# sandyz1000/face-landmark-detector

Hardware: AMD Instinct MI355X
Metric: faces/sec (whole node), 256x256 batch inference: fused preprocess + FCN-8 forward + softmax + top-4 landmark decode + similarity/alignment warp (higher is better)
Workload: dtype f32; 1 GPU; BASELINE configs[1]: batch=64/GPU 256x256x3 uint8 crops, fcn_8(68) vanilla encoder fp32, random-init weights (seed 2), decode top-4 thresh 0, align to 256x256; global_batch=64, parallelism=dp1

## Files before the change

face-landmark-detector_amd/build.py:

```python
from __future__ import annotations

import concurrent.futures
import hashlib
import os
import shutil
import subprocess
import sys

HERE = os.path.dirname(os.path.abspath(__file__))
ROOT = os.path.dirname(HERE)
CSRC = os.path.join(HERE, "csrc")
INCLUDE = os.path.join(ROOT, "include")
OBJ_DIR = os.path.join(HERE, "csrc", "build")
LIB_PATH = os.path.join(HERE, "libflm_hip.so")

SOURCES = [
    "flm_api.hip",
    "flm_pack.hip",
    "flm_enc1.hip",
    "flm_igemm.hip",
    "flm_igemm_bf16.hip",
    "flm_conv3_halo.hip",
    "flm_score1x1.hip",
    "flm_tail_bf16.hip",
    "flm_convt.hip",
    "flm_up3_wreg.hip",
    "flm_decode.hip",
    "flm_cand.hip",
    "flm_misc.hip",
    "flm_frames.hip",
    "flm_mobile.hip",
]
FLAGS = ["--offload-arch=gfx950", "-O3", "-fPIC", "-std=c++17", "-ffp-contract=off",
         "-Wall", "-Wno-unused-function", "-I", INCLUDE, "-I", CSRC]


FILE_FLAGS = {"flm_enc1.hip": ["-mllvm", "-amdgpu-mfma-vgpr-form"]}


def _hipcc() -> str:
    for c in (shutil.which("hipcc"), "/opt/rocm/bin/hipcc"):
        if c and os.path.exists(c):
            return c
    raise RuntimeError("hipcc not found: the HIP extension cannot be built")


def _stamp(paths) -> str:
    h = hashlib.sha256()
    h.update(" ".join(FLAGS).encode())
    h.update(repr(sorted(FILE_FLAGS.items())).encode())
    for p in sorted(paths):
        with open(p, "rb") as f:
            h.update(p.encode())
            h.update(f.read())
    return h.hexdigest()


def build(force: bool = False, verbose: bool = True, extra_flags=()) -> str:
    os.makedirs(OBJ_DIR, exist_ok=True)
    headers = [os.path.join(CSRC, f) for f in os.listdir(CSRC) if f.endswith(".h")] + \
              [os.path.join(INCLUDE, f) for f in os.listdir(INCLUDE) if f.endswith(".h")]
    srcs = [os.path.join(CSRC, s) for s in SOURCES]
    stamp = _stamp(srcs + headers) + " ".join(extra_flags)
    stamp_file = os.path.join(OBJ_DIR, "stamp.txt")
    if not force and os.path.exists(LIB_PATH) and os.path.exists(stamp_file) and open(stamp_file).read() == stamp:
        return LIB_PATH
    hipcc = _hipcc()

    def compile_one(src):
        obj = os.path.join(OBJ_DIR, os.path.basename(src) + ".o")
        cmd = [hipcc, *FLAGS, *FILE_FLAGS.get(os.path.basename(src), []), *extra_flags, "-c", src, "-o", obj]
        r = subprocess.run(cmd, capture_output=True, text=True)
        if r.returncode != 0:
            raise RuntimeError("hipcc failed on %s:\n%s\n%s" % (src, r.stdout, r.stderr))
        if verbose and r.stderr.strip():
            sys.stderr.write(r.stderr)
        return obj
# ... 17 lines not shown
```

face-landmark-detector_amd/csrc/flm_api.hip:

```cpp
#include <cstdarg>
#include <cstdio>
#include <cstring>

#include "flm_common.h"

namespace flm {

static thread_local char g_err[512] = "";

void set_error(const char* fmt, ...) {
  va_list ap;
  va_start(ap, fmt);
  vsnprintf(g_err, sizeof(g_err), fmt, ap);
  va_end(ap);
}

int hip_fail(hipError_t e, const char* what) {
  set_error("HIP error %d (%s) at %s", (int)e, hipGetErrorString(e), what);
  return FLM_ERR_HIP;
}

struct ProfRec {
  const char* name;
  hipEvent_t a, b;
// ... 92 lines not shown
    if (fc_bytes > W.splitk_bytes) W.splitk_bytes = fc_bytes;
  }
  if (n <= 4) {
    const size_t enc3_bytes = sizeof(float) * 4 * (size_t)4 * (h / 4) * (w / 4) * 256;
    if (enc3_bytes > W.splitk_bytes) W.splitk_bytes = enc3_bytes;
  }
  W.splitk = take(cur, W.splitk_bytes);
  W.oh = h + (A.fcn32 ? 32 : 8);
  W.ow = w + (A.fcn32 ? 32 : 8);
  W.probs = SIZE_MAX;
  W.decode = SIZE_MAX;
  W.sub = W.tau = W.cand = W.cand_cnt = SIZE_MAX;
  W.cand_cap = 0;
  if (out_mode == FLM_OUT_LANDMARKS) {
    W.probs = take(cur, sizeof(float) * (size_t)n * W.oh * W.ow * C);
    W.decode = take(cur, decode_ws_bytes(n, W.oh, W.ow, C, decode_mode, n_points));
    if (landmark_candidates_enabled(co, g, A.fcn32, decode_mode, n_points, W.oh, W.ow)) {
      const int h3 = h / 8, w3 = w / 8;
      W.sub = take(cur, sizeof(unsigned) * (size_t)n * convt_sample_slots(g, h3, w3, cand_sub_for(co, n_points, g.bf16 != 0)) * 16 * g.MT);
      W.tau = take(cur, sizeof(float) * (size_t)n * C);
      W.cand_cap = (int)align_up((size_t)C * 64 * n_points * 4 / co.cap_div, 64);
      if (W.cand_cap < 64) W.cand_cap = 64;
      W.cand = take(cur, sizeof(unsigned long long) * (size_t)n * W.cand_cap);
      W.cand_cnt = take(cur, sizeof(unsigned) * ((size_t)n + 1));
    }
  }
  W.total = cur;
  return W;
}

static int check_fcn8_shape(int n, int h, int w, int C, int dtype) {
  if (dtype != FLM_F32 && dtype != FLM_BF16) {
    set_error("fcn8: unknown dtype %d (FLM_F32 = 0, FLM_BF16 = 1)", dtype);
    return FLM_ERR_UNSUPPORTED;
  }
  if (n <= 0 || h <= 0 || w <= 0 || (h % 32) || (w % 32)) {
    set_error("fcn8: input must be [N>0, H, W, 3] with H and W multiples of 32 (got n=%d h=%d w=%d)", n, h, w);
    return FLM_ERR_SHAPE;
  }
  if (C < 1 || C > kMaxClasses) {
    set_error("fcn8: n_classes must be in [1,%d] (got %d)", kMaxClasses, C);
    return FLM_ERR_SHAPE;
  }
  if (n > (1 << 24) || h > (1 << 15) || w > (1 << 15) || (long long)n * (h + 32) * (w + 32) * C >= (1ll << 40)) {
    set_error("fcn8: batch too large (n=%d h=%d w=%d: at most 2^40 output values per call)", n, h, w);
    return FLM_ERR_SHAPE;
  }
  return FLM_OK;
}

static int conv_layer(hipStream_t s, const char* blob, const ConvPack& c, const void* x, void* y, int n, int h,
                      int w, int relu, int pool, int posmajor, int dtype, int out_f32 = 0,
                      float* splitk_ws = nullptr, size_t splitk_bytes = 0, int stride = 1,
                      const void* res = nullptr) {
  IgemmDesc d;
  d.bf16 = dtype == FLM_BF16;
  d.out_f32 = out_f32;
  d.stride = stride;
  d.res = res;
  d.splitk_ws = splitk_ws;
  d.splitk_ws_bytes = splitk_bytes;
  d.x = x;
  d.wt = blob + c.w;
  d.scale = reinterpret_cast<const float*>(blob + c.scale);
  d.shift = reinterpret_cast<const float*>(blob + c.shift);
  d.y = y;
  d.n = n; d.h = h; d.w = w; d.cin = c.cin;
  d.cout = c.cout; d.coutpad = c.coutpad; d.ldc = c.cout;
  d.kh = c.kh; d.kw = c.kw; d.pad = c.pad;
  d.relu = relu; d.pool = pool; d.posmajor = posmajor;
  return launch_igemm(s, d);
}

}

using namespace flm;

extern "C" {

int flm_abi_version(void) { return FLM_ABI_VERSION; }

int flm_debug_query(const char* key, int arg) {
  if (key && !strcmp(key, "igemm_occupancy")) return igemm_occupancy((size_t)arg);
  return -1;
}

int flm_set_tuning(const char* key, int value) {
  if (!key) return FLM_ERR_ARG;
  if (!strcmp(key, "none")) return FLM_OK;
  if (!strcmp(key, "bf16_big_tiles")) {
    flm::igemm_bf16_big_enable(value);
    return FLM_OK;
  }
  if (!strcmp(key, "f32_two_level")) {
    flm::igemm_f32_group(value ? 0 : -1);
    return FLM_OK;
  }
  if (!strcmp(key, "f32_lean_tile")) {
    flm::igemm_f32_lean_enable(value);
    return FLM_OK;
  }
  if (!strcmp(key, "bf16_mfma16")) {
    flm::igemm_bf16_big_m16(value);
    return FLM_OK;
  }
  if (!strcmp(key, "bf16_halo_mfma16")) {
    flm::conv3_halo_m16(value);
    return FLM_OK;
  }
  if (!strcmp(key, "bf16_lds_dma")) {
    flm::igemm_bf16_big_dma(value);
    return FLM_OK;
  }
  if (!strcmp(key, "landmark_candidates") || !strcmp(key, "candidate_sub_phases") || !strcmp(key, "candidate_cap_div")) {
    set_error("flm_set_tuning: '%s' changes the workspace layout and is a per-call option now: pass flm_forward_opts to "
              "flm_fcn_workspace_bytes_opts / flm_fcn_forward_opts", key);
    return FLM_ERR_ARG;
  }
  if (!strcmp(key, "up3_cand8")) {
    if (value < 0 || value > 7) {
      set_error("flm_set_tuning: up3_cand8 must be in [0,7]");
      return FLM_ERR_ARG;
    }
    flm::convt_cand8_enable(value);
    return FLM_OK;
  }
  if (!strcmp(key, "up3_cand8_rows")) {
    if (value < 0 || value > 8 || (value & (value - 1))) {
      set_error("flm_set_tuning: up3_cand8_rows must be 0, 1, 2, 4 or 8");
      return FLM_ERR_ARG;
    }
    flm::convt_cand8_rows(value);
    return FLM_OK;
  }
  if (!strcmp(key, "up3_wreg")) {
    if (value < 0 || value > 1) {
      set_error("flm_set_tuning: up3_wreg must be 0 or 1");
      return FLM_ERR_ARG;
    }
    flm::convt_wreg_enable(value);
    return FLM_OK;
  }
  if (!strcmp(key, "bf16_score1x1")) {
    flm::score1x1_enable(value);
    return FLM_OK;
  }
  if (!strcmp(key, "bf16_fused_tail")) {
    flm::tail_fused_enable(value);
    return FLM_OK;
  }
  if (!strcmp(key, "decode_lds_dma")) {
    flm::decode_dma_enable(value);
    return FLM_OK;
  }
  if (!strcmp(key, "posmajor_order")) {
    flm::igemm_posperm_enable(value);
    return FLM_OK;
  }
  if (!strcmp(key, "warp_rows")) {
    if (value != 0 && value != 1 && value != 4) {
      set_error("flm_set_tuning: warp_rows must be 0, 1 or 4");
      return FLM_ERR_ARG;
    }
    flm::warp_rows_enable(value);
    return FLM_OK;
  }
  if (!strcmp(key, "bf16_conv3_halo")) {
    flm::conv3_halo_enable(value);
    return FLM_OK;
  }
  if (!strcmp(key, "bf16_group_n")) {
    if (value < 0 || value > 32 || (value & (value - 1))) {
      set_error("flm_set_tuning: bf16_group_n must be 0 or a power of two <= 32");
      return FLM_ERR_ARG;
    }
    flm::igemm_bf16_group_n(value);
    return FLM_OK;
  }
  set_error("flm_set_tuning: unknown key '%s'", key);
  return FLM_ERR_ARG;
}

int flm_profile_enable(int max_records) {
  if (g_prof) return FLM_OK;
  if (max_records <= 0 || max_records > (1 << 20)) {
    set_error("flm_profile_enable: bad record count");
    return FLM_ERR_ARG;
  }
  g_prof = new ProfRec[max_records];
  for (int i = 0; i < max_records; ++i) {
    FLM_HIP(hipEventCreate(&g_prof[i].a));
    FLM_HIP(hipEventCreate(&g_prof[i].b));
  }
  g_prof_cap = max_records;
  g_prof_n = 0;
  return FLM_OK;
}

int flm_profile_reset(void) {
  g_prof_n = 0;
  return FLM_OK;
// ... 216 lines not shown
      case ENC_MB_CONV1:
        rc = launch_mb_conv1(s, xin, in_format, n, hi, wi, w0, sc0, sh0, yout, bf);
        break;
      case ENC_RN_CONV1:
        rc = launch_rn_conv1(s, xin, in_format, n, hi, wi, w0, sc0, sh0, yout, bf);
        break;
      case ENC_MAXPOOL3:
        rc = launch_maxpool3(s, xin, n, hi, wi, e.cin, yout, bf);
        break;
      case ENC_MB_DW:
        rc = launch_mb_depthwise(s, xin, n, hi, wi, e.cin, e.stride, w0, sc0, sh0, yout, bf);
        break;
      case ENC_CONV3:
        rc = conv_layer(s, blob, L.enc[i], xin, yout, n, hi, wi,  1, e.pool, 0, dtype, 0,
                        reinterpret_cast<float*>(ws + W.splitk), W.splitk_bytes);
        break;
      case ENC_MB_PW:
        if (L.enc[i].cin != e.cin) {
          int pn = n, ph = hi, pw = wi;
          if (!(pw & 1)) pw >>= 1;
          else if (!(ph & 1)) ph >>= 1;
          else if (!(pn & 1)) pn >>= 1;
          else {
            set_error("flm_fcn_forward: the paired pointwise conv needs an even number of pixels per batch");
            rc = FLM_ERR_SHAPE;
            break;
          }
          rc = conv_layer(s, blob, L.enc[i], xin, yout, pn, ph, pw,  2, 0, 0, dtype);
        } else {
          rc = conv_layer(s, blob, L.enc[i], xin, yout, n, hi, wi,  2, 0, 0, dtype);
        }
        break;
      case ENC_CONV:
        rc = conv_layer(s, blob, L.enc[i], xin, yout, n, hi, wi, e.relu, 0, 0, dtype, 0, nullptr, 0, e.stride,
                        e.res >= 0 ? ws + W.act[e.res] : nullptr);
        break;
      default:
        set_error("flm_fcn_forward: unknown encoder layer kind %d", e.kind);
        rc = FLM_ERR_ARG;
    }
    if (rc) return rc;
  }
  const int h5 = h / 32, w5 = w / 32, h4 = h / 16, w4 = w / 16, h3 = h / 8, w3 = w / 8;
  { ProfScope ps(s, "fc6");
  rc = conv_layer(s, blob, L.fc6, f[4], fc6, n, h5, w5, 1, 0,  1, dtype, 0,
                  reinterpret_cast<float*>(ws + W.splitk), W.splitk_bytes); }
  if (rc) return rc;
  { ProfScope ps(s, "fc7");
  rc = conv_layer(s, blob, L.fc7, fc6, fc7, n, h5, w5, 1, 0, 0, dtype, 0,
                  reinterpret_cast<float*>(ws + W.splitk), W.splitk_bytes); }
  if (rc) return rc;
  { ProfScope ps(s, "score5");
  rc = conv_layer(s, blob, L.score5, fc7, score5, n, h5, w5, 0, 0, 0, dtype,  1,
                  reinterpret_cast<float*>(ws + W.splitk), W.splitk_bytes); }
  if (rc) return rc;
  ConvTDesc t;
  t.g = L.g;
  t.n = n;
  if (!fcn32) {
  { ProfScope ps(s, "score4");
  rc = conv_layer(s, blob, L.score4, f[3], fuse4, n, h4, w4, 0, 0, 0, dtype, 1); }
  if (rc) return rc;
  const bool fuse_seg = bf && L.g.C == 68 && L.score3.cin == 256 && L.score3.kh == 1;
  int fused_seg = 0;
  if (!fuse_seg) {
  { ProfScope ps(s, "score3");
  rc = conv_layer(s, blob, L.score3, f[2], seg, n, h3, w3, 0, 0, 0, dtype, 1); }
  if (rc) return rc;
  }
  t.x = score5; t.wf = blob + L.up5; t.skip = fuse4; t.y = fuse4;
  t.hi = h5; t.wi = w5; t.ho = h4; t.wo = w4; t.s = 2; t.ldy = L.g.Cp; t.epilogue = 0;
  { ProfScope ps(s, "up5");
  rc = launch_convt(s, t); }
  if (rc) return rc;
  if (fuse_seg) {
    ProfScope ps(s, "seg_fused");
    fused_seg = launch_seg_fused_bf16(s, fuse4, blob + L.up4, f[2], blob + L.score3.w,
                                      reinterpret_cast<const float*>(blob + L.score3.scale),
                                      reinterpret_cast<const float*>(blob + L.score3.shift), seg, n, h4, w4, L.g.C, L.g.Cp,
                                      L.g.G, L.score3.cin, L.score3.coutpad);
    if (fused_seg < 0) return fused_seg;
  }
  if (fuse_seg && !fused_seg) {
    ProfScope ps(s, "score3");
    rc = conv_layer(s, blob, L.score3, f[2], seg, n, h3, w3, 0, 0, 0, dtype, 1);
    if (rc) return rc;
  }
  t.x = fuse4; t.wf = blob + L.up4; t.skip = seg; t.y = seg;
  t.hi = h4; t.wi = w4; t.ho = h3; t.wo = w3;
  if (!fused_seg) {
  { ProfScope ps(s, "up4");
  rc = launch_convt(s, t); }
  if (rc) return rc;
  }
  }
  t.wf = blob + L.up3; t.skip = nullptr; t.ho = W.oh; t.wo = W.ow; t.ldy = C;
  if (fcn32) { t.x = score5; t.hi = h5; t.wi = w5; t.s = 32; }
  else { t.x = seg; t.hi = h3; t.wi = w3; t.s = 8; }
  if (out_mode == FLM_OUT_LOGITS || out_mode == FLM_OUT_PROBS) {
    t.y = out_dev;
    t.epilogue = (out_mode == FLM_OUT_PROBS) ? 1 : 0;
    if (out_mode == FLM_OUT_LOGITS && (C & 3)) {
      set_error("flm_fcn8_forward: FLM_OUT_LOGITS needs n_classes %% 4 == 0");
      return FLM_ERR_UNSUPPORTED;
    }
    ProfScope ps(s, "up3");
    return launch_convt(s, t);
  }
  if (out_mode == FLM_OUT_CLASSMAP) {
    t.y = out_dev;
    t.epilogue = 2;
    ProfScope ps(s, "up3");
    return launch_convt(s, t);
  }
  float* probs = reinterpret_cast<float*>(ws + W.probs);
  const unsigned* gate = nullptr;
  if (W.cand != SIZE_MAX) {
    float* sub = reinterpret_cast<float*>(ws + W.sub);
    float* tau = reinterpret_cast<float*>(ws + W.tau);
    unsigned* cnt = reinterpret_cast<unsigned*>(ws + W.cand_cnt);
    unsigned long long* cand = reinterpret_cast<unsigned long long*>(ws + W.cand);
    FLM_HIP(hipMemsetAsync(cnt, 0, sizeof(unsigned) * ((size_t)n + 1), s));
    ConvTDesc ts = t;
    ts.y = sub; ts.epilogue = 4; ts.sub = cand_sub_for(co, n_points, L.g.bf16 != 0);
    { ProfScope ps(s, "up3_sub");
    rc = launch_convt(s, ts); }
    if (rc) return rc;
    { ProfScope ps(s, "tau");
    rc = launch_cand_tau(s, reinterpret_cast<const unsigned*>(sub), n, convt_sample_slots(L.g, t.hi, t.wi, cand_sub_for(co, n_points, L.g.bf16 != 0)), 16 * L.g.MT, C,
                         n_points, tau); }
    if (rc) return rc;
    ConvTDesc tc = t;
    tc.y = nullptr; tc.epilogue = 3; tc.tau = tau; tc.cand = cand; tc.cand_cnt = cnt; tc.cand_cap = W.cand_cap;
    tc.scratch = probs; tc.scratch_bytes = sizeof(float) * (size_t)n * W.oh * W.ow * C;
    { ProfScope ps(s, "up3");
    rc = launch_convt(s, tc); }
    if (rc) return rc;
    { ProfScope ps(s, "decode");
    rc = launch_cand_merge(s, cand, cnt, n, W.ow, C, n_points, thresh, W.cand_cap, static_cast<double*>(out_dev)); }
    if (rc) return rc;
    gate = cnt + n;
    t.gate = gate;
  }
// ... 173 lines not shown
```

face-landmark-detector_amd/csrc/flm_common.h:

```cpp
#pragma once

#include <hip/hip_runtime.h>
#include <stddef.h>
#include <stdint.h>

#include <atomic>
#include <mutex>

#include "flm.h"

namespace flm {

void set_error(const char* fmt, ...);
int hip_fail(hipError_t e, const char* what);

#define FLM_HIP(call)                                            \
  do {                                                           \
    hipError_t e_ = (call);                                      \
    if (e_ != hipSuccess) return ::flm::hip_fail(e_, #call);     \
  } while (0)

#define FLM_LAUNCH_CHECK(what)                                   \
  do {                                                           \
    hipError_t e_ = hipGetLastError();                           \
// ... 74 lines not shown
struct Fcn8Pack {
  size_t enc1_w;
  size_t enc1_scale, enc1_shift;
  ConvPack enc[kMaxEnc];
  ConvPack fc6, fc7, score5, score4, score3;
  size_t up5, up4, up3;
  ConvTGeom g;
  int dtype;
  int arch;
  ArchSpec spec;
  size_t total;
};
Fcn8Pack fcn8_pack_layout(int C, int dtype, int arch = 0);

struct Fcn8Ws {
  size_t act[kMaxEnc];
  size_t f[5];
  size_t fc6, fc7, score5, fuse4, seg;
  size_t splitk;
  size_t splitk_bytes;
  size_t probs;
  size_t decode;
  size_t sub, tau, cand, cand_cnt;
  int cand_cap;
  size_t total;
  int oh, ow;
};
Fcn8Ws fcn8_ws_layout(int n, int h, int w, int C, int dtype, int out_mode, int decode_mode, int n_points,
                      int arch = 0, const flm_forward_opts* opts = nullptr);

int launch_pack_fcn(hipStream_t s, const flm_fcn_params& p, int C, const Fcn8Pack& L, char* blob);

int launch_enc1(hipStream_t s, const void* x, int in_format, int n, int h, int w, const float* w1p,
                const float* scale, const float* shift, void* f1, int out_bf16, int pool);

struct IgemmDesc {
  const void* x;
  const void* wt;
  const float* scale;
  const float* shift;
  void* y;
  int bf16;
  int out_f32;
  int n, h, w, cin;
  int cout;
  int coutpad;
  int ldc;
  int kh, kw, pad;
  int relu, pool, posmajor;
  int stride;
  const void* res;
  float* splitk_ws;
  size_t splitk_ws_bytes;
};
int launch_igemm(hipStream_t s, const IgemmDesc& d);
int igemm_occupancy(size_t lds_bytes);
void igemm_f32_group(int steps);
void igemm_f32_lean_enable(int on);
void igemm_bf16_big_enable(int on);
void igemm_bf16_group_n(int gn);
void igemm_bf16_big_dma(int on);
void igemm_bf16_big_m16(int on);
void conv3_halo_enable(int on);
void conv3_halo_m16(int on);
void score1x1_enable(int on);
void tail_fused_enable(int on);
void decode_dma_enable(int on);
void warp_rows_enable(int on);
void igemm_posperm_enable(int on);
int launch_seg_fused_bf16(hipStream_t s, const float* fuse4, const void* w4_packed, const void* f3, const void* w3,
                          const float* scale3, const float* shift3, float* seg, int n, int h4, int w4d, int C, int Cp,
                          int G, int cin3, int coutpad3);

struct ConvTDesc {
  const float* x;
  const void* wf;
  const float* skip;
  void* y;
  int n, hi, wi;
  int ho, wo;
  int s;
  int ldy;
  int epilogue;
  ConvTGeom g;
  int sub = 0;
  const float* tau = nullptr;
  unsigned long long* cand = nullptr;
  unsigned* cand_cnt = nullptr;
  int cand_cap = 0;
  const unsigned* gate = nullptr;
  void* scratch = nullptr;
  size_t scratch_bytes = 0;
};
int launch_convt(hipStream_t s, const ConvTDesc& d);
int convt_candidates_supported(const ConvTGeom& g);
__host__ __device__ inline int convt_share_layout(const ConvTGeom& g, int s) {
  return g.C == 68 && (g.bf16 ? g.G == 9 : g.G == 17) && (s % 4) == 0;
}
int convt_sample_slots(const ConvTGeom& g, int hi, int wi, int sub);
void convt_cand8_enable(int mask);
void convt_cand8_rows(int rpw);
void convt_wreg_enable(int on);
int launch_cand_tau(hipStream_t s, const unsigned* wave_max, int n, int slots, int ld, int l, int n_points, float* tau);

int launch_mb_conv1(hipStream_t s, const void* x, int in_format, int n, int h, int w, const float* wgt,
                    const float* scale, const float* shift, void* y, int bf16);
int launch_mb_depthwise(hipStream_t s, const void* x, int n, int h, int w, int c, int stride, const float* wgt,
                        const float* scale, const float* shift, void* y, int bf16);
int launch_rn_conv1(hipStream_t s, const void* x, int in_format, int n, int h, int w, const float* wgt,
                    const float* scale, const float* shift, void* y, int bf16);
int launch_maxpool3(hipStream_t s, const void* x, int n, int h, int w, int c, void* y, int bf16);

size_t decode_ws_bytes(int n, int h, int w, int l, int mode, int n_points);
int launch_decode(hipStream_t s, const float* hm, int n, int h, int w, int l, int mode, int n_points, float thresh,
                  double* out, void* ws, size_t ws_bytes, const unsigned* gate = nullptr);
size_t decode_sweep_ws_bytes(int n, int h, int w, int l, const int* modes, int n_modes);
int launch_decode_sweep(hipStream_t s, const float* hm, int n, int h, int w, int l, const int* modes, int n_modes,
                        float thresh, double* out, void* ws, size_t ws_bytes);
int launch_gaussian_heatmaps(hipStream_t s, const double* kp, int n, int l, int h, int w, double two_sigma_sq,
                             float* out);
int launch_cand_merge(hipStream_t s, const unsigned long long* cand, unsigned* cand_cnt, int n, int w, int l,
                      int n_points, float thresh, int cap, double* out);

int launch_preprocess(hipStream_t s, const uint8_t* img, int n, int h, int w, int norm, float* out);
int launch_similarity(hipStream_t s, const double* lm, const double* tmpl, int n, int k, double sx, double sy, float* m);
// ... 20 lines not shown
```

face-landmark-detector_amd/csrc/flm_igemm.hip:

```cpp
#include <type_traits>
#include <vector>

#include "flm_igemm_args.h"

#ifndef FLM_IGEMM_VAR
#define FLM_IGEMM_VAR 0
#endif

namespace flm {

typedef float f32x16 __attribute__((ext_vector_type(16)));
typedef __bf16 bf16x8 __attribute__((ext_vector_type(8)));

constexpr int BM = 128, BN = 128, BK = 32;
constexpr int TILE_F = BM * BK;

__device__ __forceinline__ int swz(int row, int chunk) { return row * BK + ((chunk ^ ((row >> 1) & 7)) << 2); }

__device__ __forceinline__ float f4c(const float4& v, int i) { return i == 0 ? v.x : (i == 1 ? v.y : (i == 2 ? v.z : v.w)); }

template <bool BF, int IDX>
__device__ __forceinline__ void mfma_slot(const float4& a0, const float4& a1, const float4& b0, const float4& b1,
                                          f32x16& c00, f32x16& c01, f32x16& c10, f32x16& c11) {
  if constexpr (BF) {
// ... 674 lines not shown
    for (int s = 0; s < ksplit; ++s) v += part[(size_t)s * total + i];
    v = fmaf(v, scale[c], shift[c]);
    if (relu) v = fmaxf(v, 0.f);
    if (out_bf16) reinterpret_cast<unsigned short*>(y)[i] = f2bf(v);
    else reinterpret_cast<float*>(y)[i] = v;
  }
}

__global__ void splitk_reduce_pool_kernel(const float* __restrict__ part, const float* __restrict__ scale,
                                          const float* __restrict__ shift, void* __restrict__ y, int M, int ldc, int cout,
                                          int ksplit, int relu, float relu_max, int out_bf16) {
  const size_t total = (size_t)(M >> 2) * ldc, plane = (size_t)M * ldc;
  for (size_t i = (size_t)blockIdx.x * blockDim.x + threadIdx.x; i < total; i += (size_t)gridDim.x * blockDim.x) {
    const int c = (int)(i % ldc);
    if (c >= cout) continue;
    const size_t q = i / ldc;
    float best = -3.402823466e38f;
#pragma unroll
    for (int e = 0; e < 4; ++e) {
      float v = 0.f;
      for (int s = 0; s < ksplit; ++s) v += part[(size_t)s * plane + (4 * q + e) * ldc + c];
      v = fmaf(v, scale[c], shift[c]);
      if (relu) v = fminf(fmaxf(v, 0.f), relu_max);
      best = fmaxf(best, v);
    }
    if (out_bf16) reinterpret_cast<unsigned short*>(y)[i] = f2bf(best);
    else reinterpret_cast<float*>(y)[i] = best;
  }
}

int igemm_occupancy(size_t lds_bytes) {
  int nb = -1;
  if (hipOccupancyMaxActiveBlocksPerMultiprocessor(&nb, reinterpret_cast<const void*>(&igemm_kernel<false, 0, true>), 256,
                                                   lds_bytes) != hipSuccess)
    return -1;
  return nb;
}

template <bool BF, bool TWO = false>
static int dispatch(hipStream_t s, const IgemmDesc& d, const IgemmArgs& a) {
  if constexpr (TWO) {
    if (!d.posmajor && g_f32_lean.load(std::memory_order_relaxed)) {
      if (d.pool) return d.relu ? launch_t<BF, 1, true, TWO, true>(s, a) : launch_t<BF, 1, false, TWO, true>(s, a);
      return d.relu ? launch_t<BF, 0, true, TWO, true>(s, a) : launch_t<BF, 0, false, TWO, true>(s, a);
    }
  }
  if (d.pool) return d.relu ? launch_t<BF, 1, true, TWO>(s, a) : launch_t<BF, 1, false, TWO>(s, a);
  if (d.posmajor) return d.relu ? launch_t<BF, 2, true, TWO>(s, a) : launch_t<BF, 2, false, TWO>(s, a);
  return d.relu ? launch_t<BF, 0, true, TWO>(s, a) : launch_t<BF, 0, false, TWO>(s, a);
}

static std::atomic<int> g_f32_group{0};
void igemm_f32_group(int steps) { g_f32_group = steps; }

int launch_igemm(hipStream_t s, const IgemmDesc& d) {
  const int es = d.bf16 ? 2 : 4;
  const int bke = 128 / es;
  if (d.cin % bke != 0 || d.coutpad % BN != 0 || d.cout > d.coutpad || d.kh * d.kw > 64) {
    set_error("igemm: unsupported shape cin=%d coutpad=%d cout=%d k=%dx%d (%s)", d.cin, d.coutpad, d.cout, d.kh, d.kw,
              d.bf16 ? "bf16" : "fp32");
    return FLM_ERR_SHAPE;
  }
  if (d.pool && ((d.h & 1) || (d.w & 1))) {
    set_error("igemm: pooled layer needs even h,w (got %dx%d)", d.h, d.w);
    return FLM_ERR_SHAPE;
  }
  const int stride = d.stride > 0 ? d.stride : 1;
  const int ho = (d.h + 2 * d.pad - d.kh) / stride + 1, wo = (d.w + 2 * d.pad - d.kw) / stride + 1;
  if ((stride != 1 || d.res) && (d.pool || d.posmajor)) {
    set_error("igemm: stride / residual are only built for the row-major pixel order");
    return FLM_ERR_UNSUPPORTED;
  }
  if (stride == 1 && (ho != d.h || wo != d.w)) {
    set_error("igemm: stride-1 layers must be 'same' (k=%dx%d pad=%d)", d.kh, d.kw, d.pad);
    return FLM_ERR_SHAPE;
  }
  const long long M = (long long)d.n * ho * wo;
  if (M <= 0 || M > (1ll << 30)) {
    set_error("igemm: pixel count %lld out of range", M);
    return FLM_ERR_SHAPE;
  }
  if ((long long)d.n * d.h * d.w * d.cin * es >= (1ll << 32) || (long long)d.coutpad * d.kh * d.kw * d.cin >= (1ll << 31)) {
    set_error("igemm: tensor exceeds the 32-bit offset range (split the batch)");
    return FLM_ERR_SHAPE;
  }
  IgemmArgs a;
  a.x = d.x; a.wt = d.wt; a.scale = d.scale; a.shift = d.shift; a.y = d.y;
  a.out_f32 = d.bf16 ? d.out_f32 : 1;
  a.relu_max = d.relu == 2 ? 6.0f : 3.402823466e38f;
  a.n = d.n; a.h = d.h; a.w = d.w; a.cin = d.cin; a.cout = d.cout; a.ldc = d.ldc;
  a.ho = ho; a.wo = wo; a.stride = stride; a.res = d.res;
  a.kh = d.kh; a.kw = d.kw; a.pad = d.pad;
  a.M = (int)M;
  a.K = d.kh * d.kw * d.cin;
  a.mtiles = cdiv(a.M, BM);
  a.cpt = d.cin / bke;
  a.kw_magic = (65536 + d.kw - 1) / d.kw;
  a.ksplit = 1;
  a.gm = a.gn = 1;
  a.grp_magic = 0;
  a.posperm_on = 0;
  for (int k = 0; k < 8; ++k) a.posperm[k] = 0ull;
  a.dx = a.dy = 1;
  a.dx_magic = a.dy_magic = 1u << 30;
  a.dx_shift = a.dy_shift = 0;
  a.all_taps = 0;
// ... 9 lines not shown
    int ks = (tiles <= 64 || narrow_1x1) ? 8 : (tiles <= 128 ? 4 : 2);
    if (few_faces && tiles > 16 * faces) ks = 8;
    int per = d.kh * d.kw == 1 ? 8 : 1;
    if (d.kh * d.kw == 1 && tiles <= 8) {
      ks = 32;
      per = 4;
    }
    if (d.kh * d.kw > 1) {
      if (ks > d.kh * d.kw * a.cpt / 8) ks = d.kh * d.kw * a.cpt / 8;
    } else if (ks > a.cpt / per) {
      ks = a.cpt / per;
    }
    const size_t part_rows = few_faces ? (size_t)(a.M / faces) * 4 : (size_t)a.M;
    if (ks > 1 && (size_t)ks * part_rows * d.ldc * sizeof(float) <= d.splitk_ws_bytes) {
      a.ksplit = ks;
      a.part = d.splitk_ws;
    }
  }
  a.ntiles = cdiv(d.cout, BN);
  if (d.bf16) {
    const int sk = launch_score1x1_bf16(s, a, d.relu, d.pool, d.posmajor, d.coutpad);
    if (sk < 0) return sk;
    if (sk == 1) return FLM_OK;
    const int halo = launch_conv3_halo_bf16(s, a, d.relu, d.pool, d.posmajor);
    if (halo < 0) return halo;
    if (halo == 1) return FLM_OK;
    const int big = launch_igemm_bf16_big(s, a, d.relu, d.pool, d.posmajor, d.coutpad);
    if (big < 0) return big;
    if (big == 1) return FLM_OK;
  }
  int rc;
  const int f32_knob = g_f32_group.load(std::memory_order_relaxed);
  if (d.bf16) {
    rc = dispatch<true>(s, d, a);
  } else if (f32_knob < 0) {
    rc = dispatch<false>(s, d, a);
  } else {
    const int dense = d.kh * d.kw * a.cpt;
    if (dense >= 8192) {
      set_error("igemm: %d k-steps per output exceed the group divider's range", dense);
      return FLM_ERR_SHAPE;
    }
    int grp = 2;
    while ((grp + 1) * (grp + 1) <= dense) ++grp;
    a.grp_magic = (65536 + grp - 1) / grp;
    const long long face_in = (long long)d.h * d.w * d.cin * 4,
                    face_out = (long long)(d.pool ? (ho / 2) * (wo / 2) : ho * wo) * d.ldc * 4;
    const long long lim = (1ll << 31) - (1ll << 22);
    if (face_in >= lim) {
      set_error("igemm: one face exceeds the 2 GiB buffer range of the fp32 kernel");
      return FLM_ERR_SHAPE;
    }
    const int max_faces = (int)(lim / face_in);
    if (d.n <= max_faces) {
      rc = dispatch<false, true>(s, d, a);
    } else {
      if (a.ksplit > 1) {
        set_error("igemm: batch slicing is not built for split-K layers");
        return FLM_ERR_UNSUPPORTED;
      }
      rc = FLM_OK;
      for (int f0 = 0; f0 < d.n && rc == FLM_OK; f0 += max_faces) {
        IgemmArgs b = a;
        b.n = d.n - f0 < max_faces ? d.n - f0 : max_faces;
        b.x = reinterpret_cast<const char*>(a.x) + (size_t)f0 * face_in;
        b.y = reinterpret_cast<char*>(a.y) + (size_t)f0 * face_out;
        if (a.res) b.res = reinterpret_cast<const char*>(a.res) + (size_t)f0 * face_out;
        b.M = b.n * ho * wo;
        b.mtiles = cdiv(b.M, BM);
        rc = dispatch<false, true>(s, d, b);
      }
    }
  }
  if (rc || a.ksplit <= 1) return rc;
  const size_t total = (size_t)a.M * d.ldc;
  const int blocks = (int)((total + 255) / 256 < 2048 ? (total + 255) / 256 : 2048);
  if (d.pool) {
    splitk_reduce_pool_kernel<<<blocks, 256, 0, s>>>(a.part, a.scale, a.shift, a.y, a.M, d.ldc, d.cout, a.ksplit, d.relu,
                                                     a.relu_max, d.bf16 && !d.out_f32);
    FLM_LAUNCH_CHECK("splitk_reduce_pool_kernel");
    return FLM_OK;
  }
  splitk_reduce_kernel<<<blocks, 256, 0, s>>>(a.part, a.scale, a.shift, a.y, a.M, d.ldc, d.cout, a.ksplit, d.relu,
                                              d.bf16 && !d.out_f32);
  FLM_LAUNCH_CHECK("splitk_reduce_kernel");
  return FLM_OK;
}

}
```

Measured before the change: 7755 faces/s.

## Fuse fp32 FCN-8 tail score convs into upsample kernels and add thin score5 GEMM

Adds an fp32 fused tail kernel that computes the 1x1 score4/score3 classifier on the skip features and the stride-2 transposed-conv upsample in one pass. This removes the separate score conv launches and the intermediate skip-buffer round trips. It also adds a dedicated split-K kernel for the score5 1x1 conv (K=4096, 68 classes) in place of the generic implicit GEMM. Both paths are on by default with toggles, but are narrowly specialised to C=68, K=256 and the current packing, and must reproduce the generic kernels' summation order.

```diff
diff --git a/face-landmark-detector_amd/build.py b/face-landmark-detector_amd/build.py
--- a/face-landmark-detector_amd/build.py
+++ b/face-landmark-detector_amd/build.py
@@ -23,6 +23,7 @@
     "flm_conv3_halo.hip",
     "flm_score1x1.hip",
     "flm_tail_bf16.hip",
+    "flm_tail_f32.hip",
     "flm_convt.hip",
     "flm_up3_wreg.hip",
     "flm_decode.hip",
diff --git a/face-landmark-detector_amd/csrc/flm_api.hip b/face-landmark-detector_amd/csrc/flm_api.hip
--- a/face-landmark-detector_amd/csrc/flm_api.hip
+++ b/face-landmark-detector_amd/csrc/flm_api.hip
@@ -168,8 +168,9 @@
 static int conv_layer(hipStream_t s, const char* blob, const ConvPack& c, const void* x, void* y, int n, int h,
                       int w, int relu, int pool, int posmajor, int dtype, int out_f32 = 0,
                       float* splitk_ws = nullptr, size_t splitk_bytes = 0, int stride = 1,
-                      const void* res = nullptr) {
+                      const void* res = nullptr, int thin = 0) {
   IgemmDesc d;
+  d.thin = thin;
   d.bf16 = dtype == FLM_BF16;
   d.out_f32 = out_f32;
   d.stride = stride;
@@ -198,6 +199,7 @@
 
 int flm_debug_query(const char* key, int arg) {
   if (key && !strcmp(key, "igemm_occupancy")) return igemm_occupancy((size_t)arg);
+  if (key && !strcmp(key, "score5_thin_launches")) return score5_thin_f32_launches();
   return -1;
 }
 
@@ -263,6 +265,14 @@
   }
   if (!strcmp(key, "bf16_fused_tail")) {
     flm::tail_fused_enable(value);
+    return FLM_OK;
+  }
+  if (!strcmp(key, "f32_fused_tail")) {
+    flm::tail_f32_fused_enable(value);
+    return FLM_OK;
+  }
+  if (!strcmp(key, "f32_score5_thin")) {
+    flm::score5_thin_f32_enable(value);
     return FLM_OK;
   }
   if (!strcmp(key, "decode_lds_dma")) {
@@ -585,25 +595,35 @@
   if (rc) return rc;
   { ProfScope ps(s, "score5");
   rc = conv_layer(s, blob, L.score5, fc7, score5, n, h5, w5, 0, 0, 0, dtype,  1,
-                  reinterpret_cast<float*>(ws + W.splitk), W.splitk_bytes); }
+                  reinterpret_cast<float*>(ws + W.splitk), W.splitk_bytes, 1, nullptr,  1); }
   if (rc) return rc;
   ConvTDesc t;
   t.g = L.g;
   t.n = n;
   if (!fcn32) {
+  const bool tail_f32 = !bf && tail_fused_f32_applies(L.g, L.score4, n, h5, w5) && tail_fused_f32_applies(L.g, L.score3, n, h4, w4);
+  const bool fuse4_f32 = tail_f32, seg_f32 = tail_f32;
+  if (!fuse4_f32) {
   { ProfScope ps(s, "score4");
   rc = conv_layer(s, blob, L.score4, f[3], fuse4, n, h4, w4, 0, 0, 0, dtype, 1); }
   if (rc) return rc;
+  }
   const bool fuse_seg = bf && L.g.C == 68 && L.score3.cin == 256 && L.score3.kh == 1;
   int fused_seg = 0;
-  if (!fuse_seg) {
+  if (!fuse_seg && !seg_f32) {
   { ProfScope ps(s, "score3");
   rc = conv_layer(s, blob, L.score3, f[2], seg, n, h3, w3, 0, 0, 0, dtype, 1); }
   if (rc) return rc;
   }
   t.x = score5; t.wf = blob + L.up5; t.skip = fuse4; t.y = fuse4;
   t.hi = h5; t.wi = w5; t.ho = h4; t.wo = w4; t.s = 2; t.ldy = L.g.Cp; t.epilogue = 0;
-  { ProfScope ps(s, "up5");
+  if (fuse4_f32) {
+    ProfScope ps(s, "fuse4_fused");
+    rc = launch_tail_fused_f32(s, score5, blob + L.up5, f[3], blob + L.score4.w,
+                               reinterpret_cast<const float*>(blob + L.score4.scale),
+                               reinterpret_cast<const float*>(blob + L.score4.shift), fuse4, n, h5, w5);
+  } else {
+  ProfScope ps(s, "up5");
   rc = launch_convt(s, t); }
   if (rc) return rc;
   if (fuse_seg) {
@@ -621,7 +641,13 @@
   }
   t.x = fuse4; t.wf = blob + L.up4; t.skip = seg; t.y = seg;
   t.hi = h4; t.wi = w4; t.ho = h3; t.wo = w3;
-  if (!fused_seg) {
+  if (seg_f32) {
+    ProfScope ps(s, "seg_fused");
+    rc = launch_tail_fused_f32(s, fuse4, blob + L.up4, f[2], blob + L.score3.w,
+                               reinterpret_cast<const float*>(blob + L.score3.scale),
+                               reinterpret_cast<const float*>(blob + L.score3.shift), seg, n, h4, w4);
+    if (rc) return rc;
+  } else if (!fused_seg) {
   { ProfScope ps(s, "up4");
   rc = launch_convt(s, t); }
   if (rc) return rc;
diff --git a/face-landmark-detector_amd/csrc/flm_common.h b/face-landmark-detector_amd/csrc/flm_common.h
--- a/face-landmark-detector_amd/csrc/flm_common.h
+++ b/face-landmark-detector_amd/csrc/flm_common.h
@@ -150,10 +150,12 @@
   const void* res;
   float* splitk_ws;
   size_t splitk_ws_bytes;
+  int thin = 0;
 };
 int launch_igemm(hipStream_t s, const IgemmDesc& d);
 int igemm_occupancy(size_t lds_bytes);
 void igemm_f32_group(int steps);
+int igemm_f32_group_get();
 void igemm_f32_lean_enable(int on);
 void igemm_bf16_big_enable(int on);
 void igemm_bf16_group_n(int gn);
@@ -163,12 +165,22 @@
 void conv3_halo_m16(int on);
 void score1x1_enable(int on);
 void tail_fused_enable(int on);
+void tail_f32_fused_enable(int on);
 void decode_dma_enable(int on);
 void warp_rows_enable(int on);
 void igemm_posperm_enable(int on);
 int launch_seg_fused_bf16(hipStream_t s, const float* fuse4, const void* w4_packed, const void* f3, const void* w3,
                           const float* scale3, const float* shift3, float* seg, int n, int h4, int w4d, int C, int Cp,
                           int G, int cin3, int coutpad3);
+
+bool tail_fused_f32_applies(const ConvTGeom& g, const ConvPack& cls, int n, int hi, int wi);
+int launch_tail_fused_f32(hipStream_t s, const float* x, const void* wt_packed, const void* f, const void* wc,
+                          const float* scale, const float* shift, float* y, int n, int hi, int wi);
+
+bool score5_thin_f32_applies(int M, int K, int cout, int ldc, int ksplit);
+int launch_score5_thin_f32(hipStream_t s, const void* x, const void* wc, float* part, int M, int grp_magic);
+void score5_thin_f32_enable(int on);
+int score5_thin_f32_launches();
 
 struct ConvTDesc {
   const float* x;
diff --git a/face-landmark-detector_amd/csrc/flm_igemm.hip b/face-landmark-detector_amd/csrc/flm_igemm.hip
--- a/face-landmark-detector_amd/csrc/flm_igemm.hip
+++ b/face-landmark-detector_amd/csrc/flm_igemm.hip
@@ -750,6 +750,7 @@
 
 static std::atomic<int> g_f32_group{0};
 void igemm_f32_group(int steps) { g_f32_group = steps; }
+int igemm_f32_group_get() { return g_f32_group.load(std::memory_order_relaxed); }
 
 int launch_igemm(hipStream_t s, const IgemmDesc& d) {
   const int es = d.bf16 ? 2 : 4;
@@ -865,7 +866,10 @@
       return FLM_ERR_SHAPE;
     }
     const int max_faces = (int)(lim / face_in);
-    if (d.n <= max_faces) {
+    if (d.thin && d.kh * d.kw == 1 && stride == 1 && !d.res && !d.pool && !d.posmajor && !d.relu &&
+        score5_thin_f32_applies(a.M, a.K, d.cout, d.ldc, a.ksplit)) {
+      rc = launch_score5_thin_f32(s, a.x, a.wt, a.part, a.M, a.grp_magic);
+    } else if (d.n <= max_faces) {
       rc = dispatch<false, true>(s, d, a);
     } else {
       if (a.ksplit > 1) {
diff --git a/face-landmark-detector_amd/csrc/flm_tail_f32.hip b/face-landmark-detector_amd/csrc/flm_tail_f32.hip
--- /dev/null
+++ b/face-landmark-detector_amd/csrc/flm_tail_f32.hip
@@ -0,0 +1,374 @@
+#include "flm_convt_dev.h"
+
+namespace flm {
+
+namespace tail32 {
+constexpr int C = 68, MT = 5, G = 17, K = 256, STEPS = K / 32, WAVES = 8;
+constexpr int SUBG = 6;
+constexpr int PHASE_F4 = G * MT * 64;
+constexpr int PIECES = G * MT;
+constexpr int CLS_STEP_F4 = 2 * 4 * 64, CLS4_STEP_F4 = 2 * 16;
+constexpr int CLS_F4 = STEPS * CLS_STEP_F4;
+constexpr int CLS4_F4 = STEPS * CLS4_STEP_F4;
+constexpr int AFF_F = 160;
+constexpr size_t LDS_BYTES = sizeof(float4) * (PHASE_F4 + CLS_F4 + CLS4_F4) + sizeof(float) * AFF_F;
+static_assert(LDS_BYTES <= 160 * 1024, "tail32: one workgroup per CU");
+constexpr int K5 = 4096, KS5 = 8, STEPS5 = K5 / 32 / KS5;
+constexpr size_t LDS5_BYTES = sizeof(float4) * STEPS5 * (CLS_STEP_F4 + CLS4_STEP_F4);
+static_assert(LDS5_BYTES <= 160 * 1024, "tail32: one workgroup per CU");
+
+#define TAIL32_PIN(x) asm volatile("" : "+v"(x))
+
+template <int NSTEP>
+__device__ __forceinline__ void cls_fill(float4* lds, const float* __restrict__ wc, int ldk, int k0, int tid) {
+  constexpr int MAIN = NSTEP * CLS_STEP_F4, TOTAL = MAIN + NSTEP * CLS4_STEP_F4;
+  constexpr int PER = (TOTAL + 64 * WAVES - 1) / (64 * WAVES), B = PER > 9 ? 9 : PER;
+#pragma unroll
+  for (int it0 = 0; it0 < PER; it0 += B) {
+    f32x4 lo[B], hi[B];
+#pragma unroll
+    for (int b = 0; b < B; ++b) {
+      const int i = tid + 64 * WAVES * (it0 + b), ic = i < TOTAL ? i : TOTAL - 1;
+      const bool main = ic < MAIN;
+      const int j = ic - MAIN;
+      const int dt = main ? ic >> 8 : j >> 4;
+      const int cls = main ? 16 * ((ic >> 6) & 3) + (ic & 15) : 64 + ((j >> 2) & 3);
+      const int qq = main ? (ic >> 4) & 3 : j & 3;
+      const float* row = wc + (size_t)cls * ldk + k0 + 16 * dt + 4 * (qq & 1);
+      lo[b] = *reinterpret_cast<const f32x4*>(row);
+      hi[b] = *reinterpret_cast<const f32x4*>(row + 8);
+    }
+#pragma unroll
+    for (int b = 0; b < B; ++b) {
+      const int i = tid + 64 * WAVES * (it0 + b);
+      const bool o = ((i < MAIN ? i >> 4 : i - MAIN) & 2) != 0;
+      const float4 v = make_float4(o ? lo[b][1] : lo[b][0], o ? lo[b][3] : lo[b][2], o ? hi[b][1] : hi[b][0], o ? hi[b][3] : hi[b][2]);
+      if (it0 + b < PER && i < TOTAL) lds[i] = v;
+    }
+  }
+}
+
+__device__ __forceinline__ void cls_step(const float4* wl3, const float4* wl34, const float4 (&fa)[4], bool odd, f32x4 (&acc)[MT]) {
+  const f32x4 zero4 = (f32x4){0.f, 0.f, 0.f, 0.f};
+#pragma unroll
+  for (int tp = 0; tp < 2; ++tp) {
+    float4 af[MT];
+#pragma unroll
+    for (int m = 0; m < 4; ++m) af[m] = wl3[(tp * 4 + m) * 64];
+    af[4] = wl34[tp * 16];
+#pragma unroll
+    for (int tt = 0; tt < 2; ++tt) {
+      const float4 fq = fa[2 * tp + tt];
+      const float b0v = odd ? fq.y : fq.x, b1v = odd ? fq.w : fq.z;
+#pragma unroll
+      for (int m = 0; m < MT; ++m)
+        acc[m] = __builtin_amdgcn_mfma_f32_16x16x4f32(tt ? af[m].z : af[m].x, b0v, (tp == 0 && tt == 0) ? zero4 : acc[m], 0, 0, 0);
+#pragma unroll
+      for (int m = 0; m < MT; ++m)
+        acc[m] = __builtin_amdgcn_mfma_f32_16x16x4f32(tt ? af[m].w : af[m].y, b1v, acc[m], 0, 0, 0);
+    }
+  }
+}
+}
+
+__global__ __launch_bounds__(64 * tail32::WAVES, 1) void tail_fused_f32_kernel(const float* __restrict__ x,
+                                                                               const float4* __restrict__ wt,
+                                                                               const float* __restrict__ f,
+                                                                               const float* __restrict__ wc,
+                                                                               const float* __restrict__ scale,
+                                                                               const float* __restrict__ shift,
+                                                                               float* __restrict__ y,
+                                                                               int n, int hi, int wi) {
+  using namespace tail32;
+  extern __shared__ __attribute__((aligned(16))) char smem_raw[];
+  float4* ldsT = reinterpret_cast<float4*>(smem_raw);
+  float4* ldsC = ldsT + PHASE_F4;
+  float* aff = reinterpret_cast<float*>(ldsC + CLS_F4 + CLS4_F4);
+  const int tid = threadIdx.x, lane = tid & 63;
+  const int wave = __builtin_amdgcn_readfirstlane(tid >> 6);
+  const int r = lane & 15, q = lane >> 4;
+  const int phase = blockIdx.x & 3, a0 = phase >> 1, b0 = phase & 1;
+  const int wb = blockIdx.x >> 2, nbp = gridDim.x >> 2;
+  const int hw = hi * wi, P = n * hw;
+  const int slices = (P + 15) >> 4;
+  const int wo = 2 * wi;
+
+  const bool odd = (q >> 1) != 0;
+  float4 fv[STEPS][4];
+#define TAIL32_LOAD_FV(D0, D1)                                                                                 \
+  _Pragma("unroll") for (int d_ = (D0); d_ < (D1); ++d_) _Pragma("unroll") for (int t_ = 0; t_ < 4; ++t_)      \
+    fv[d_][t_] = *reinterpret_cast<const float4*>(fr + 32 * d_ + 8 * t_);
+  const int sl_first = wb * WAVES + wave, sl_stride = nbp * WAVES;
+  {
+    typedef __attribute__((address_space(3))) char lds_char;
+    const unsigned lds0 = (unsigned)(size_t)((lds_char*)smem_raw);
+    const unsigned long long wbase = reinterpret_cast<unsigned long long>(wt + (size_t)phase * PHASE_F4);
+    const cand8::dma_srd wsrd = (cand8::dma_srd){(int)(unsigned)wbase, (int)(unsigned)((wbase >> 32) & 0xffffu), PHASE_F4 * 16, 0x00020000};
+#pragma unroll
+    for (int k = 0; k < (PIECES + WAVES - 1) / WAVES; ++k) {
+      const int pc = wave + WAVES * k;
+      if (pc < PIECES) cand8::dma_piece(wsrd, lds0 + (unsigned)pc * 1024u, (unsigned)lane * 16u, pc * 1024);
+    }
+  }
+  cls_fill<STEPS>(ldsC, wc, K, 0, tid);
+  for (int i = tid; i < AFF_F; i += 64 * WAVES) {
+    const int c = i < 80 ? i : i - 80;
+    aff[i] = c < C ? (i < 80 ? scale[c] : shift[c]) : 0.f;
+  }
+  __builtin_amdgcn_s_waitcnt(0x0f70);
+  __syncthreads();
+
+  const f32x4 zero4 = (f32x4){0.f, 0.f, 0.f, 0.f};
+  const __amdgpu_buffer_rsrc_t xsrd = __builtin_amdgcn_make_buffer_rsrc(const_cast<float*>(x), 0, P * (C * 4), 0x00020000);
+  const float4* wl3 = ldsC + lane;
+  const float4* wl34 = ldsC + CLS_F4 + (r >> 2) * 4 + q;
+  for (int sl = sl_first; sl < slices; sl += sl_stride) {
+    const int p = 16 * sl + r;
+    const bool pv = p < P;
+    const int pc = pv ? p : P - 1;
+    const int img = pc / hw, rem = pc - img * hw;
+    const int i0 = rem / wi, j0 = rem - i0 * wi;
+    const size_t opix = ((size_t)img * 2 * hi + (2 * i0 + a0)) * wo + (2 * j0 + b0);
+
+    const float* fr = f + opix * K + 4 * (q & 1);
+    TAIL32_LOAD_FV(0, 4)
+    __builtin_amdgcn_sched_barrier(0);
+    f32x4 acc[MT], sum[MT], top[MT];
+    f32x4 xf[G];
+#pragma unroll
+    for (int m = 0; m < MT; ++m) acc[m] = sum[m] = top[m] = zero4;
+#pragma unroll
+    for (int d = 0; d < STEPS; ++d) {
+#pragma unroll
+      for (int m = 0; m < MT; ++m) {
+        sum[m] += acc[m];
+        TAIL32_PIN(sum[m]);
+      }
+      cls_step(wl3 + d * CLS_STEP_F4, wl34 + d * CLS4_STEP_F4, fv[d], odd, acc);
+      if (d < STEPS / 2) {
+        __builtin_amdgcn_sched_barrier(0);
+        TAIL32_LOAD_FV(d + 4, d + 5)
+        __builtin_amdgcn_sched_barrier(0);
+      }
+      if (d == STEPS / 2 - 1) {
+        __builtin_amdgcn_sched_barrier(0);
+        int qv = q;
+        asm volatile("" : "+v"(qv));
+        const unsigned pix_off = (unsigned)(pc * (C * 4));
+#pragma unroll
+        for (int g = 0; g < G; ++g) {
+          const int k0 = 16 * g + 4 * qv;
+          const int tap = k0 / C, c = k0 - tap * C;
+          const int di = tap >> 1, dj = tap & 1;
+          const bool ok = i0 >= di && j0 >= dj;
+          const unsigned off = ok ? pix_off - (unsigned)((di * wi + dj) * (C * 4)) + (unsigned)(4 * c) : 0x80000000u;
+          xf[g] = __builtin_bit_cast(f32x4, __builtin_amdgcn_raw_buffer_load_b128(xsrd, off, 0, 0));
+        }
+        __builtin_amdgcn_sched_barrier(0);
+      }
+      if (d > 0 && (d & 1) == 0) {
+#pragma unroll
+        for (int m = 0; m < MT; ++m) {
+          top[m] += sum[m];
+          TAIL32_PIN(top[m]);
+          sum[m] = zero4;
+        }
+      }
+    }
+    f32x4 skip[MT];
+#pragma unroll
+    for (int m = 0; m < MT; ++m) {
+      const f32x4 v = top[m] + (sum[m] + acc[m]);
+      if (m < 4) {
+        const float4 sc = *reinterpret_cast<const float4*>(aff + 16 * m + 4 * q);
+        const float4 sh = *reinterpret_cast<const float4*>(aff + 80 + 16 * m + 4 * q);
+        skip[m] = (f32x4){fmaf(v[0], sc.x, sh.x), fmaf(v[1], sc.y, sh.y), fmaf(v[2], sc.z, sh.z), fmaf(v[3], sc.w, sh.w)};
+      } else {
+        skip[m] = (f32x4){fmaf(v[0], aff[64 + q], aff[80 + 64 + q]), 0.f, 0.f, 0.f};
+      }
+      TAIL32_PIN(skip[m]);
+    }
+
+    f32x4 ct[MT], sub[MT];
+#pragma unroll
+    for (int m = 0; m < MT; ++m) ct[m] = sub[m] = zero4;
+#pragma unroll
+    for (int g = 0; g < G; ++g) {
+      float4 af[MT];
+#pragma unroll
+      for (int m = 0; m < MT; ++m) af[m] = ldsT[(g * MT + m) * 64 + lane];
+      const bool sub_first = g % SUBG == 0, sub_last = g == G - 1 || (g + 1) % SUBG == 0;
+      if (g < SUBG) {
+#pragma unroll
+        for (int m = 0; m < MT; ++m) ct[m] = __builtin_amdgcn_mfma_f32_16x16x4f32(af[m].x, xf[g][0], ct[m], 0, 0, 0);
+#pragma unroll
+        for (int m = 0; m < MT; ++m) ct[m] = __builtin_amdgcn_mfma_f32_16x16x4f32(af[m].y, xf[g][1], ct[m], 0, 0, 0);
+#pragma unroll
+        for (int m = 0; m < MT; ++m) ct[m] = __builtin_amdgcn_mfma_f32_16x16x4f32(af[m].z, xf[g][2], ct[m], 0, 0, 0);
+#pragma unroll
+        for (int m = 0; m < MT; ++m) ct[m] = __builtin_amdgcn_mfma_f32_16x16x4f32(af[m].w, xf[g][3], ct[m], 0, 0, 0);
+      } else {
+#pragma unroll
+        for (int m = 0; m < MT; ++m) sub[m] = __builtin_amdgcn_mfma_f32_16x16x4f32(af[m].x, xf[g][0], sub_first ? zero4 : sub[m], 0, 0, 0);
+#pragma unroll
+        for (int m = 0; m < MT; ++m) sub[m] = __builtin_amdgcn_mfma_f32_16x16x4f32(af[m].y, xf[g][1], sub[m], 0, 0, 0);
+#pragma unroll
+        for (int m = 0; m < MT; ++m) sub[m] = __builtin_amdgcn_mfma_f32_16x16x4f32(af[m].z, xf[g][2], sub[m], 0, 0, 0);
+#pragma unroll
+        for (int m = 0; m < MT; ++m) sub[m] = __builtin_amdgcn_mfma_f32_16x16x4f32(af[m].w, xf[g][3], sub[m], 0, 0, 0);
+        if (sub_last) {
+#pragma unroll
+          for (int m = 0; m < MT; ++m) {
+            ct[m] += sub[m];
+            TAIL32_PIN(ct[m]);
+          }
+        }
+      }
+    }
+
+    if (pv) {
+      float* yp = y + opix * C;
+#pragma unroll
+      for (int m = 0; m < 4; ++m) {
+        const f32x4 v = ct[m] + skip[m];
+        *reinterpret_cast<float4*>(yp + 16 * m + 4 * q) = make_float4(v[0], v[1], v[2], v[3]);
+      }
+      yp[64 + q] = ct[4][0] + skip[4][0];
+    }
+  }
+#undef TAIL32_LOAD_FV
+}
+
+__global__ __launch_bounds__(64 * tail32::WAVES, 1) void score5_thin_f32_kernel(const float* __restrict__ x,
+                                                                                const float* __restrict__ wc,
+                                                                                float* __restrict__ part,
+                                                                                int M, int grp_magic) {
+  using namespace tail32;
+  extern __shared__ __attribute__((aligned(16))) char smem_raw[];
+  float4* ldsC = reinterpret_cast<float4*>(smem_raw);
+  const int tid = threadIdx.x, lane = tid & 63;
+  const int wave = __builtin_amdgcn_readfirstlane(tid >> 6);
+  const int r = lane & 15, q = lane >> 4;
+  const int ks = blockIdx.y, d0 = ks * STEPS5;
+  const int slices = (M + 15) >> 4;
+  const bool odd = (q >> 1) != 0;
+  float4 fv[STEPS5][4];
+  constexpr int AHEAD = 4;
+#define TAIL32_LOAD_ROW(FR, D) \
+  _Pragma("unroll") for (int t_ = 0; t_ < 4; ++t_) fv[D][t_] = *reinterpret_cast<const float4*>((FR) + 32 * (D) + 8 * t_);
+  const int sl_first = blockIdx.x * WAVES + wave, sl_stride = gridDim.x * WAVES;
+  const float* fr;
+  {
+    const int sl = sl_first < slices ? sl_first : slices - 1;
+    const int p = 16 * sl + r, pc = p < M ? p : M - 1;
+    fr = x + (size_t)pc * K5 + 32 * d0 + 4 * (q & 1);
+  }
+  cls_fill<STEPS5>(ldsC, wc, K5, 32 * d0, tid);
+#pragma unroll
+  for (int d = 0; d < AHEAD; ++d) TAIL32_LOAD_ROW(fr, d)
+  __syncthreads();
+
+  const f32x4 zero4 = (f32x4){0.f, 0.f, 0.f, 0.f};
+  const float4* wl3 = ldsC + lane;
+  const float4* wl34 = ldsC + STEPS5 * CLS_STEP_F4 + (r >> 2) * 4 + q;
+  for (int sl = sl_first; sl < slices; sl += sl_stride) {
+    const int p = 16 * sl + r;
+    f32x4 acc[MT], sum[MT], top[MT];
+#pragma unroll
+    for (int m = 0; m < MT; ++m) acc[m] = sum[m] = top[m] = zero4;
+    const int sln = sl + sl_stride < slices ? sl + sl_stride : slices - 1;
+    const int pn = 16 * sln + r, pcn = pn < M ? pn : M - 1;
+    const float* frn = x + (size_t)pcn * K5 + 32 * d0 + 4 * (q & 1);
+    const bool more = sl + sl_stride < slices;
+#pragma unroll
+    for (int it = 0; it < STEPS5; ++it) {
+#pragma unroll
+      for (int m = 0; m < MT; ++m) {
+        sum[m] += acc[m];
+        TAIL32_PIN(sum[m]);
+      }
+      cls_step(wl3 + it * CLS_STEP_F4, wl34 + it * CLS4_STEP_F4, fv[it], odd, acc);
+      __builtin_amdgcn_sched_barrier(0);
+      if (it + AHEAD < STEPS5) {
+        TAIL32_LOAD_ROW(fr, it + AHEAD)
+      } else if (more) {
+        TAIL32_LOAD_ROW(frn, it + AHEAD - STEPS5)
+      }
+      __builtin_amdgcn_sched_barrier(0);
+      if (it > 0 && (((d0 + it - 1) * grp_magic) >> 16) != (((d0 + it) * grp_magic) >> 16)) {
+#pragma unroll
+        for (int m = 0; m < MT; ++m) {
+          top[m] += sum[m];
+          TAIL32_PIN(top[m]);
+          sum[m] = zero4;
+        }
+      }
+    }
+    fr = frn;
+    if (p < M) {
+      float* yp = part + ((size_t)ks * M + p) * C;
+#pragma unroll
+      for (int m = 0; m < 4; ++m) {
+        const f32x4 v = top[m] + (sum[m] + acc[m]);
+        *reinterpret_cast<float4*>(yp + 16 * m + 4 * q) = make_float4(v[0], v[1], v[2], v[3]);
+      }
+      yp[64 + q] = top[4][0] + (sum[4][0] + acc[4][0]);
+    }
+  }
+#undef TAIL32_LOAD_ROW
+}
+
+#undef TAIL32_PIN
+
+static std::atomic<int> g_f32_fused_tail{1};
+void tail_f32_fused_enable(int on) { g_f32_fused_tail.store(on, std::memory_order_relaxed); }
+
+bool tail_fused_f32_applies(const ConvTGeom& g, const ConvPack& cls, int n, int hi, int wi) {
+  using namespace tail32;
+  if (!g_f32_fused_tail.load(std::memory_order_relaxed) || igemm_f32_group_get() != 0) return false;
+  if (g.bf16 || g.C != C || g.Cp != C || g.G != G || g.MT != MT) return false;
+  if (cls.cin != K || cls.kh != 1 || cls.kw != 1 || cls.cout != C || cls.coutpad < C) return false;
+  return n >= 1 && hi >= 1 && wi >= 1 && (long long)n * hi * wi * (C * 4) < (1ll << 31);
+}
+
+static std::atomic<int> g_f32_score5_thin{1};
+void score5_thin_f32_enable(int on) { g_f32_score5_thin.store(on, std::memory_order_relaxed); }
+
+bool score5_thin_f32_applies(int M, int K, int cout, int ldc, int ksplit) {
+  using namespace tail32;
+  return g_f32_score5_thin.load(std::memory_order_relaxed) && K == K5 && cout == C && ldc == C && ksplit == KS5 && M >= 1 &&
+         M < (1 << 26);
+}
+
+static std::atomic<int> g_score5_thin_launches{0};
+int score5_thin_f32_launches() { return g_score5_thin_launches.load(std::memory_order_relaxed); }
+
+int launch_score5_thin_f32(hipStream_t s, const void* x, const void* wc, float* part, int M, int grp_magic) {
+  using namespace tail32;
+  g_score5_thin_launches.fetch_add(1, std::memory_order_relaxed);
+  static FuncAttrOnce attr;
+  FLM_FUNC_ATTR_ONCE(attr, (&score5_thin_f32_kernel), LDS5_BYTES);
+  int gx = cdiv(cdiv(M, 16), WAVES);
+  if (gx > 256 / KS5) gx = 256 / KS5;
+  score5_thin_f32_kernel<<<dim3(gx, KS5), 64 * WAVES, LDS5_BYTES, s>>>(static_cast<const float*>(x), static_cast<const float*>(wc),
+                                                                      part, M, grp_magic);
+  FLM_LAUNCH_CHECK("score5_thin_f32_kernel");
+  return FLM_OK;
+}
+
+int launch_tail_fused_f32(hipStream_t s, const float* x, const void* wt_packed, const void* f, const void* wc,
+                          const float* scale, const float* shift, float* y, int n, int hi, int wi) {
+  using namespace tail32;
+  static FuncAttrOnce attr;
+  FLM_FUNC_ATTR_ONCE(attr, (&tail_fused_f32_kernel), LDS_BYTES);
+  const long long slices = ((long long)n * hi * wi + 15) / 16;
+  long long per_phase = (slices + WAVES - 1) / WAVES;
+  if (per_phase > 64) per_phase = 64;
+  tail_fused_f32_kernel<<<dim3((unsigned)(4 * per_phase)), 64 * WAVES, LDS_BYTES, s>>>(
+      x, static_cast<const float4*>(wt_packed), static_cast<const float*>(f), static_cast<const float*>(wc), scale, shift, y,
+      n, hi, wi);
+  FLM_LAUNCH_CHECK("tail_fused_f32_kernel");
+  return FLM_OK;
+}
+
+}
```

Result: no change. 7824 faces/s, median of 6 (+0.9%).
